# chorowski-lab/pytorch-asr

Hardware: AMD Instinct MI355X
Metric: CTC train-step frames/sec (higher is better)
Workload: dtype bf16; 1 GPU; WSJ mono-char CTC (egs/wsj/yamls/ctc.yaml shapes), DeepSpeech2 conv+4xBiLSTM-320 encoder + FSTDecoder, fwd+bwd+GradientClipping(clip 480000, skip 4.8e+06 = recipe x global_batch/16)+PolyakDecay+Adam, synthetic 40-dim x 1-channel x 1000-frame fbank; batch_per_gpu=768, global_batch=768, frames=1000, classes=49, parallelism=dp1, batch_norm=per-replica statistics, optimizer_steps=142, step_boundary=device: att_speech.fused_step (clip / skip decision + Adam, no read-back)

## Files before the change

### pytorch-asr_amd/csrc/lstm.hip

```cpp
#include "common.h"
#include "../../include/asr_amd.h"
#include "recurrence.h"
#include <stdlib.h>

namespace {

__device__ __forceinline__ void lstm_cell_fwd(const float pre[4], float cprev, float gate[4],
                                              float &c, float &h) {
#pragma clang fp contract(off)
    gate[0] = sigmoidf_(pre[0]);
    gate[1] = sigmoidf_(pre[1]);
    gate[2] = tanhf_(pre[2]);
    gate[3] = sigmoidf_(pre[3]);
    c = gate[1] * cprev + gate[0] * gate[2];
    h = gate[3] * tanhf_(c);
}

typedef float f32x2 __attribute__((ext_vector_type(2)));
__device__ __forceinline__ f32x2 sigmoid2_(f32x2 x) {
#pragma clang fp contract(off)
    const f32x2 t = x * -1.4426950408889634f;
    f32x2 e = {__builtin_amdgcn_exp2f(t.x), __builtin_amdgcn_exp2f(t.y)};
    e = e + 1.f;
    return f32x2{__builtin_amdgcn_rcpf(e.x), __builtin_amdgcn_rcpf(e.y)};
}
__device__ __forceinline__ f32x2 tanh2_(f32x2 x) {
#pragma clang fp contract(off)
    const f32x2 t = x * -2.8853900817779268f;
    f32x2 e = {__builtin_amdgcn_exp2f(t.x), __builtin_amdgcn_exp2f(t.y)};
    e = e + 1.f;
    const f32x2 r = {__builtin_amdgcn_rcpf(e.x), __builtin_amdgcn_rcpf(e.y)};
    return r * 2.f - 1.f;
}
__device__ __forceinline__ void lstm_cell_fwd2(const f32x2 pre[4], f32x2 cprev, f32x2 gate[4],
                                               f32x2 &c, f32x2 &h) {
#pragma clang fp contract(off)
    gate[0] = sigmoid2_(pre[0]);
    gate[1] = sigmoid2_(pre[1]);
    gate[2] = tanh2_(pre[2]);
    gate[3] = sigmoid2_(pre[3]);
    c = gate[1] * cprev + gate[0] * gate[2];
    h = gate[3] * tanh2_(c);
}

__device__ __forceinline__ void lstm_cell_bwd(const float g[4], float cs, float cp, float dh,
                                              float dcin, float d[4], float &dcout) {
#pragma clang fp contract(off)
    const float gi = g[0], gf = g[1], gg = g[2], go = g[3];
    const float tc = tanhf_(cs);
    const float dc = dh * go * (1.f - tc * tc) + dcin;
    d[3] = dh * tc * go * (1.f - go);
    d[0] = dc * gg * gi * (1.f - gi);
    d[1] = dc * cp * gf * (1.f - gf);
    d[2] = dc * gi * (1.f - gg * gg);
    dcout = dc * gf;
}

template <int GXB>
__device__ __forceinline__ float load_gx(const void *gx, size_t i) {
    if constexpr (GXB) return (float)((const __bf16 *)gx)[i];
    else return ((const float *)gx)[i];
}

struct LstmFwdParams {
    const void *gx;
    int gx_bf16;
    const __bf16 *x;
    const __bf16 *wih;
    const __bf16 *whh;
    const int32_t *lens;
    int T, B, H;
    __bf16 *hbuf;
    float *cbuf;
    float *y;
    __bf16 *ybf;
    u32x2 *gates;
    float *csave;
    int step;
    int s_begin, s_end;
    __bf16 *xsum;
};


#ifdef ASR_LSTM_STAMPS
#define STAMP(i) stamp[i] = __builtin_amdgcn_s_memtime()
#else
#define STAMP(i) do {} while (0)
#endif

template <int KS, int BT, int GXB>
__global__ __launch_bounds__(256) void lstm_fwd_step_kernel(LstmFwdParams p) {
#ifdef ASR_LSTM_STAMPS
    unsigned long long stamp[4];
    const unsigned long long stamp_start = __builtin_amdgcn_s_memtime();
#endif
    __shared__ __attribute__((aligned(16))) __bf16 a_lds[BT * KS * 512];
    __shared__ float g_lds[BT][4][32][33];
    const int H = p.H, B = p.B;
    const int j0 = blockIdx.x * 32, b0 = blockIdx.y * 32 * BT, dir = blockIdx.z;
    const int wave = threadIdx.x >> 6, lane = threadIdx.x & 63;
    const int t = dir == 0 ? p.step : p.T - 1 - p.step;
    const int Bp = (B + 63) & ~63;
    const __bf16 *hprev = p.hbuf + ((size_t)(p.step & 1) * 2 + dir) * Bp * H;
    __bf16 *hnext = p.hbuf + ((size_t)((p.step + 1) & 1) * 2 + dir) * Bp * H;

    bf16x8 fb[KS];
    {
        const __bf16 *bp = p.whh + ((size_t)(dir * 4 + wave) * H * H) +
// ... 69 lines not shown
        const int bt = rowg >> 5, row = rowg & 31;
        const int b = b0 + rowg, j = j0 + col;
        if (b < B) {
            const size_t sidx = ((size_t)dir * B + b) * H + j;
            float *yo = p.y + (((size_t)t * B + b) * 2 + dir) * H + j;
            __bf16 *ybo = p.ybf + (((size_t)dir * (p.T + 2) + t + 1) * B + b) * H + j;
            const size_t csv = (((size_t)t * 2 + dir) * B + b) * H + j;
            if (pact[e]) {
                float pre[4], gt[4], c, h;
#pragma unroll
                for (int g = 0; g < 4; ++g) pre[g] = g_lds[bt][g][row][col] + pgx[e][g];
                lstm_cell_fwd(pre, pc[e], gt, c, h);
                p.cbuf[sidx] = c;
                hnext[frag_off(b, j, KS)] = (__bf16)h;
                if (p.y) *yo = h;
                *ybo = (__bf16)h;
                p.gates[csv] = pack_gates(gt);
                p.csave[csv] = c;
            } else {
                hnext[frag_off(b, j, KS)] = hprev[frag_off(b, j, KS)];
                if (p.y) *yo = 0.f;
                *ybo = (__bf16)0.f;
                p.csave[csv] = pc[e];
            }
        }
    }
    STAMP(3);
#ifdef ASR_LSTM_STAMPS
    __syncthreads();
    if (threadIdx.x == 0 && b0 < B) {
        float *o = p.y + (((size_t)t * B + b0) * 2 + dir) * H + j0;
        o[0] = (float)(stamp[0] - stamp_start);
        for (int i = 1; i < 4; ++i) o[i] = (float)(stamp[i] - stamp[i - 1]);
    }
#endif
}

struct LstmBwdParams {
    const float *dy;
    int dy_shared;
    const __bf16 *wihT;
    float *dx;
    const __bf16 *whhT;
    const int32_t *lens;
    int T, B, H;
    const u32x2 *gates;
    const float *csave;
    __bf16 *dgbuf;
    float *dcbuf;
    __bf16 *dgates;
    int step;
};

template <int KS, int BT>
__global__ __launch_bounds__(256) void lstm_bwd_step_kernel(LstmBwdParams p) {
    __shared__ float part[BT][4][32][33];
    const int H = p.H, B = p.B, H4 = 4 * p.H;
    const int j0 = blockIdx.x * 32, b0 = blockIdx.y * 32 * BT, dir = blockIdx.z;
    const int wave = threadIdx.x >> 6, lane = threadIdx.x & 63;
    const int t = dir == 0 ? p.T - 1 - p.step : p.step;
    const int Bp = (B + 63) & ~63;
    constexpr int KS4 = 4 * KS;
    const __bf16 *dgprev = p.dgbuf + ((size_t)(p.step & 1) * 2 + dir) * Bp * H4;
    __bf16 *dgnext = p.dgbuf + ((size_t)((p.step + 1) & 1) * 2 + dir) * Bp * H4;

    bf16x8 fb[KS], fa[BT][KS];
    {
        const __bf16 *bp = p.whhT + (size_t)dir * H * H4 +
                           (((size_t)blockIdx.x * KS4 + (size_t)wave * KS) * 64 + lane) * 8;
#pragma unroll
        for (int k = 0; k < KS; ++k) fb[k] = *reinterpret_cast<const bf16x8 *>(bp + k * 512);
#pragma unroll
        for (int bt = 0; bt < BT; ++bt) {
            const __bf16 *ap = dgprev + ((((size_t)blockIdx.y * BT + bt) * KS4 +
                                          (size_t)wave * KS) * 64 + lane) * 8;
#pragma unroll
            for (int k = 0; k < KS; ++k)
                fa[bt][k] = *reinterpret_cast<const bf16x8 *>(ap + k * 512);
        }
    }

    constexpr int NE = 4 * BT;
    float pg[NE][4], pcs[NE], pcp[NE], pdy[NE], pdc[NE];
    bool pact[NE];
#pragma unroll
    for (int e = 0; e < NE; ++e) {
        const int idx = e * 256 + threadIdx.x;
        const int b = b0 + (idx >> 5), j = j0 + (idx & 31);
        const int bc = b < B ? b : B - 1;
        const int len = p.lens[bc];
        pact[e] = b < B && t < len;
        unpack_gates(p.gates[(((size_t)t * 2 + dir) * B + bc) * H + j], pg[e]);
        pcs[e] = p.csave[(((size_t)t * 2 + dir) * B + bc) * H + j];
        const int tp = dir == 0 ? t - 1 : t + 1;
        const int tpc = tp < 0 ? 0 : (tp >= p.T ? p.T - 1 : tp);
        const float cpv = p.csave[(((size_t)tpc * 2 + dir) * B + bc) * H + j];
        pcp[e] = (tp >= 0 && tp < len) ? cpv : 0.f;
        pdy[e] = p.dy[p.dy_shared ? ((size_t)t * B + bc) * H + j : (((size_t)t * B + bc) * 2 + dir) * H + j];
        pdc[e] = p.dcbuf[((size_t)dir * B + bc) * H + j];
    }

    {
        const int col = lane & 31;
#pragma unroll
        for (int bt = 0; bt < BT; ++bt) {
            f32x16 acc;
#pragma unroll
            for (int i = 0; i < 16; ++i) acc[i] = 0.f;
#pragma unroll
            for (int k = 0; k < KS; ++k)
                acc = __builtin_amdgcn_mfma_f32_32x32x16_bf16(fa[bt][k], fb[k], acc, 0, 0, 0);
#pragma unroll
            for (int i = 0; i < 16; ++i) {
                const int row = (i & 3) + 8 * (i >> 2) + 4 * (lane >> 5);
                part[bt][wave][row][col] = acc[i];
            }
        }
    }
    __syncthreads();

#pragma unroll
    for (int e = 0; e < NE; ++e) {
        const int idx = e * 256 + threadIdx.x;
        const int rowg = idx >> 5, col = idx & 31;
        const int bt = rowg >> 5, row = rowg & 31;
        const int b = b0 + rowg, j = j0 + col;
        if (b < B) {
            const size_t sidx = ((size_t)dir * B + b) * H + j;
            __bf16 *dgo = p.dgates + (((size_t)t * B + b) * 2 + dir) * H4 + j;
            if (pact[e]) {
                const float dh = pdy[e] + (part[bt][0][row][col] + part[bt][1][row][col]) +
                                 (part[bt][2][row][col] + part[bt][3][row][col]);
                float d[4], dcout;
                lstm_cell_bwd(pg[e], pcs[e], pcp[e], dh, pdc[e], d, dcout);
                const float d_i = d[0], d_f = d[1], d_g = d[2], d_o = d[3];
                p.dcbuf[sidx] = dcout;
                dgo[0] = (__bf16)d_i; dgo[H] = (__bf16)d_f;
                dgo[2 * H] = (__bf16)d_g; dgo[3 * H] = (__bf16)d_o;
                dgnext[frag_off(b, j, KS4)] = (__bf16)d_i;
                dgnext[frag_off(b, H + j, KS4)] = (__bf16)d_f;
                dgnext[frag_off(b, 2 * H + j, KS4)] = (__bf16)d_g;
                dgnext[frag_off(b, 3 * H + j, KS4)] = (__bf16)d_o;
            } else {
                p.dcbuf[sidx] = 0.f;
                dgo[0] = (__bf16)0.f; dgo[H] = (__bf16)0.f;
                dgo[2 * H] = (__bf16)0.f; dgo[3 * H] = (__bf16)0.f;
                dgnext[frag_off(b, j, KS4)] = (__bf16)0.f;
                dgnext[frag_off(b, H + j, KS4)] = (__bf16)0.f;
                dgnext[frag_off(b, 2 * H + j, KS4)] = (__bf16)0.f;
                dgnext[frag_off(b, 3 * H + j, KS4)] = (__bf16)0.f;
            }
        }
    }
}


#ifdef ASR_LSTM_STAMPS
#define PSTAMP_DECL unsigned long long pst[6] = {0, 0, 0, 0, 0, 0}, plast = __builtin_amdgcn_s_memtime()
#define PSTAMP(i) do { const unsigned long long now_ = __builtin_amdgcn_s_memtime(); \
                       pst[i] += now_ - plast; plast = now_; } while (0)
#else
#define PSTAMP_DECL do {} while (0)
#define PSTAMP(i) do {} while (0)
#endif

typedef __attribute__((ext_vector_type(4))) int rsrc_words;
__device__ __forceinline__ rsrc_words raw_rsrc(const void *base, unsigned bytes) {
    const unsigned long long a = (unsigned long long)base;
    rsrc_words r;
    r.x = __builtin_amdgcn_readfirstlane((int)(unsigned)a);
    r.y = __builtin_amdgcn_readfirstlane((int)((unsigned)(a >> 32) & 0xffffu));
    r.z = __builtin_amdgcn_readfirstlane((int)bytes);
    r.w = 0x00020000;
    return r;
}
__device__ __forceinline__ void dma16_s(rsrc_words r, unsigned lds_byte, unsigned voff, unsigned soff) {
    unsigned keep;
    asm volatile("s_mov_b32 %0, m0\n\ts_mov_b32 m0, %1\n\ts_nop 0\n\t"
                 "buffer_load_dwordx4 %2, %3, %4 offen lds\n\ts_mov_b32 m0, %0"
                 : "=&s"(keep)
                 : "s"(lds_byte), "v"(voff), "s"(r), "s"(soff)
                 : "memory");
}
__device__ __forceinline__ void dma16_sc1(rsrc_words r, unsigned lds_byte, unsigned voff, unsigned soff) {
    unsigned keep;
// ... 360 lines not shown
                    pre[g] = f32x2{g_lds[g][row][col], g_lds[g][row + 8][col]};
                    if constexpr (!XF) pre[g] = pre[g] + f32x2{pgx[XF ? 0 : e][g], pgx[XF ? 0 : e + 1][g]};
                }
                lstm_cell_fwd2(pre, f32x2{c[e], c[e + 1]}, og, cn, hn);
                const float og0[4] = {og[0].x, og[1].x, og[2].x, og[3].x}, og1[4] = {og[0].y, og[1].y, og[2].y, og[3].y};
                sog[e] = pack_gates(og0);
                sog[e + 1] = pack_gates(og1);
                c[e] = cn.x; c[e + 1] = cn.y;
                soh[e] = dead ? __builtin_nanf("") : hn.x;
                soh[e + 1] = dead ? __builtin_nanf("") : hn.y;
                hq[e] = (__bf16)soh[e]; hq[e + 1] = (__bf16)soh[e + 1];
                shq[e] = hq[e]; shq[e + 1] = hq[e + 1];
            } else {
                cell_one(e);
                if (e + 1 < NE) cell_one(e + 1);
            }
        }
#pragma unroll
        for (int e = 0; e < NE; ++e) {
            const int row = e * 8 + wave;
            sc[e] = c[e];
            h_lds[(((col >> 4) * 64) + row + 32 * ((col >> 3) & 1)) * 8 + (col & 7)] = hq[e];
        }
        __syncthreads();
        if (wave < 4) {
            const u32x4 v = reinterpret_cast<const u32x4 *>(h_lds)[wave * 64 + lane];
            const unsigned off = (unsigned)(((((size_t)((step + 1) & 1) * 2 + dir) * Bp * H) +
                                             ((size_t)btile * KS + 4 * jt + wave) * 512 + lane * 8) * 2);
            __builtin_amdgcn_raw_buffer_store_b128(v, hres, (lane & 31) < 8 * NE ? off : 0xFFFFFFFFu,
                                                   0, ASR_SC1);
        }
        PSTAMP(3);
        bulk_store(true);
        asm volatile("s_waitcnt vmcnt(%0)" ::"n"((NOY ? 3 : 4) * NE) : "memory");
        __syncthreads();
        PSTAMP(4);
        if (tid == 0) __hip_atomic_fetch_add(myctr, 1u, __ATOMIC_RELAXED, __HIP_MEMORY_SCOPE_AGENT);
        if constexpr (summ) sum_store();
        if constexpr (!XF) {
#pragma unroll
            for (int e = 0; e < NE; ++e)
#pragma unroll
                for (int g = 0; g < 4; ++g) pgx[e][g] = ngx[e][g];
        }
        PSTAMP(5);
    }
#ifdef ASR_LSTM_STAMPS
    __syncthreads();
    if (tid == 0 && b0 < B)
        for (int i = 0; i < 6; ++i) p.y[(((size_t)0 * B + b0) * 2 + dir) * H + j0 + i] = (float)pst[i] / T;
#endif
}

template <int KS, int NE>
__global__ __launch_bounds__(512) void lstm_bwd_persist_kernel(LstmBwdParams p, LstmTeamCtl ctl) {
    extern __shared__ __attribute__((aligned(16))) unsigned char smem[];
    constexpr int KS4 = 4 * KS;
    __bf16 *a_lds = reinterpret_cast<__bf16 *>(smem);
    float (*part)[32][65] = reinterpret_cast<float (*)[32][65]>(smem + KS4 * 1024);
    __bf16 *dg_lds = reinterpret_cast<__bf16 *>(smem + KS4 * 1024 + ASR_GLDS_BYTES);
    __shared__ int dead_s;
    const int H = p.H, B = p.B, T = p.T, H4 = 4 * p.H;
    int jt = blockIdx.x, btile = blockIdx.y + ctl.bt0, dir = blockIdx.z;
    if (ctl.xcd_teams) {
        const int slot = blockIdx.x >> 3, team = (slot / (p.H / 64)) * 8 + (blockIdx.x & 7);
        if (team >= ctl.xcd_teams) return;
        jt = slot % (p.H / 64);
        btile = (team >> 1) + ctl.bt0;
        dir = team & 1;
    }
    const int j0 = jt * 64, b0 = btile * (8 * NE), njt = H / 64;
    const int tid = threadIdx.x, wave = tid >> 6, lane = tid & 63;
    const int kq = wave >> 1, js = wave & 1;
    const size_t Bp = ctl.rows;
    unsigned *myctr = ctl.ctr + ((size_t)dir * ctl.nbt + btile) * 32;
    if (tid == 0) dead_s = 0;
    for (int i = tid; i < 8192; i += 512) dg_lds[i] = (__bf16)0.f;
    for (int i = tid; i < KS4 * 64; i += 512)
        reinterpret_cast<u32x4 *>(a_lds)[i] = u32x4{0u, 0u, 0u, 0u};

    bf16x8 fb[KS];
    {
        const __bf16 *bp = p.whhT + (size_t)dir * H * H4 +
                           (((size_t)(2 * jt + js) * KS4 + (size_t)kq * KS) * 64 + lane) * 8;
#pragma unroll
        for (int k = 0; k < KS; ++k) fb[k] = *reinterpret_cast<const bf16x8 *>(bp + k * 512);
    }
    const __amdgpu_buffer_rsrc_t dres = __builtin_amdgcn_make_buffer_rsrc(
        p.dgbuf, 0, (int)(2 * 2 * Bp * H4 * 2), 0x00020000);

    const int col = lane, j = j0 + col;
    float dcarry[NE];
    int len[NE], bcl[NE];
#pragma unroll
    for (int e = 0; e < NE; ++e) {
        const int b = b0 + e * 8 + wave;
        dcarry[e] = 0.f;
        len[e] = b < B ? p.lens[b] : 0;
        bcl[e] = b < B ? b : B - 1;
    }

    typedef unsigned int u32;
    constexpr u32 OOBV = 0xFFFFFFFFu;
    u32 vcs[NE], vdy[NE], vdg[NE];
#pragma unroll
    for (int e = 0; e < NE; ++e) {
        const int b = b0 + e * 8 + wave;
        vcs[e] = (u32)((dir * B + bcl[e]) * H + j) * 4u;
        vdy[e] = (u32)(p.dy_shared ? bcl[e] * H + j : (bcl[e] * 2 + dir) * H + j) * 4u;
        vdg[e] = b < B ? (u32)((b * 2 + dir) * H4 + j) * 2u : OOBV;
    }
    const u32 fg = (u32)B * 2u * H * 8u, fcs = (u32)B * 2u * H * 4u;
    const u32 fdy = (u32)B * H * 4u * (p.dy_shared ? 1u : 2u), fdg = (u32)B * 2u * H4 * 2u;
    const u32 dy2 = p.dy_shared == 2 ? (u32)T * fdy : 0x80000000u;
    const __amdgpu_buffer_rsrc_t gR = __builtin_amdgcn_make_buffer_rsrc(
        const_cast<u32x2 *>(p.gates), 0, (int)((u32)T * fg), 0x00020000);
    const __amdgpu_buffer_rsrc_t csR = __builtin_amdgcn_make_buffer_rsrc(
        const_cast<float *>(p.csave), 0, (int)((u32)T * fcs), 0x00020000);
    const __amdgpu_buffer_rsrc_t dyR = __builtin_amdgcn_make_buffer_rsrc(
        const_cast<float *>(p.dy), 0,
        __builtin_amdgcn_readfirstlane((int)((u32)T * fdy * (p.dy_shared == 2 ? 2u : 1u))), 0x00020000);
    const __amdgpu_buffer_rsrc_t dgR = __builtin_amdgcn_make_buffer_rsrc(
        p.dgates, 0, (int)((u32)T * fdg), 0x00020000);
    auto ldf = [&](__amdgpu_buffer_rsrc_t R, u32 voff, u32 soff) -> float {
        return __builtin_bit_cast(float, __builtin_amdgcn_raw_buffer_load_b32(R, voff, soff, 0));
    };
    struct Pre { u32x2 g[NE]; float cp[NE], dy[NE], dyb[NE]; };
    auto fetch = [&](int t, Pre &q) {
        const int tp = dir == 0 ? t - 1 : t + 1;
        const int tpc = tp < 0 ? 0 : (tp >= T ? T - 1 : tp);
#pragma unroll
        for (int e = 0; e < NE; ++e) {
            q.g[e] = __builtin_amdgcn_raw_buffer_load_b64(gR, vcs[e] * 2u, (u32)t * fg, 0);
            q.cp[e] = ldf(csR, vcs[e], (u32)tpc * fcs);
            q.dy[e] = ldf(dyR, vdy[e], (u32)t * fdy);
            q.dyb[e] = ldf(dyR, vdy[e], (u32)t * fdy + dy2);
        }
    };
    Pre cur;
    float pcs[NE];
    {
        const int t0 = dir == 0 ? T - 1 : 0;
        fetch(t0, cur);
#pragma unroll
        for (int e = 0; e < NE; ++e) pcs[e] = ldf(csR, vcs[e], (u32)t0 * fcs);
    }
    __bf16 sod[NE][4] = {};
    int st = 0;
    auto bulk_store = [&](bool live) {
#pragma unroll
        for (int e = 0; e < NE; ++e)
#pragma unroll
            for (int g = 0; g < 4; ++g)
                __builtin_amdgcn_raw_buffer_store_b16(
                    (short)__builtin_bit_cast(unsigned short, sod[e][g]), dgR, live ? vdg[e] : OOBV,
                    (u32)st * fdg + (u32)g * H * 2u, 0);
    };

    PSTAMP_DECL;
    for (int step = 0; step < T; ++step) {
        const int t = dir == 0 ? T - 1 - step : step;
        if (step > 0 && tid == 0 && !dead_s) {
            if (!team_wait(myctr, (unsigned)(njt * step), ctl.spin_limit, ctl.err)) dead_s = 1;
        }
        PSTAMP(0);
        __syncthreads();
        constexpr int RL = 8 * NE, CPK = 2 * RL;
        constexpr int CHO = (KS4 - 16) * CPK, NI = (CHO + 511) / 512;
        u32x4 tmp[NI > 0 ? NI : 1];
        if constexpr (NI > 0) {
            const unsigned base = (unsigned)((((size_t)(step & 1) * 2 + dir) * Bp * H4 +
                                              (size_t)btile * KS4 * 512) * 2);
#pragma unroll
            for (int i = 0; i < NI; ++i) {
                const int co = i * 512 + tid;
                const int cc = co < CHO ? co : CHO - 1;
                const int kq = cc / CPK, q = cc - kq * CPK, g = kq / (KS - 4), r = kq - g * (KS - 4);
                const int k = g * KS + (r < 4 * jt ? r : r + 4);
                tmp[i] = __builtin_amdgcn_raw_buffer_load_b128(
                    dres, base + (k * 64 + (q < RL ? q : q + (32 - RL))) * 16, 0, ASR_SC1);
            }
        }
        bulk_store(step > 0);
#pragma unroll
        for (int i = 0; i < 2; ++i) {
            const int c = i * 512 + tid, bi = c >> 6;
            reinterpret_cast<u32x4 *>(a_lds)[((bi >> 2) * KS + 4 * jt + (bi & 3)) * 64 + (c & 63)] =
                reinterpret_cast<const u32x4 *>(dg_lds)[c];
        }
        if constexpr (NI > 0) {
#pragma unroll
            for (int i = 0; i < NI; ++i) {
                const int co = i * 512 + tid;
                const int kq = co / CPK, q = co - kq * CPK, g = kq / (KS - 4), r = kq - g * (KS - 4);
                const int k = g * KS + (r < 4 * jt ? r : r + 4);
                if (co < CHO)
                    reinterpret_cast<u32x4 *>(a_lds)[k * 64 + (q < RL ? q : q + (32 - RL))] = tmp[i];
            }
        }
        __syncthreads();
        PSTAMP(1);
        Pre nxt;
        {
            const int sn = step + 1 < T ? step + 1 : step;
            fetch(dir == 0 ? T - 1 - sn : sn, nxt);
        }
        {
            f32x16 acc;
#pragma unroll
            for (int i = 0; i < 16; ++i) acc[i] = 0.f;
            const bf16x8 *al = reinterpret_cast<const bf16x8 *>(a_lds) + (size_t)kq * KS * 64 + lane;
            acc = mfma_chain<0, KS, 4>(al, fb, acc);
            const int c32 = lane & 31;
#pragma unroll
            for (int i = 0; i < 16; ++i) {
                const int row = (i & 3) + 8 * (i >> 2) + 4 * (lane >> 5);
                part[kq][row][js * 32 + c32] = acc[i];
            }
        }
        __syncthreads();
        PSTAMP(2);
        const bool dead = dead_s != 0;
        st = t;
        const int tp = dir == 0 ? t - 1 : t + 1;
#pragma unroll
        for (int e = 0; e < NE; ++e) {
            const int row = e * 8 + wave;
            float od[4];
            if (t < len[e]) {
                const float dh = (cur.dy[e] + cur.dyb[e]) + (part[0][row][col] + part[1][row][col]) +
                                 (part[2][row][col] + part[3][row][col]);
                const float cp = (tp >= 0 && tp < len[e]) ? cur.cp[e] : 0.f;
                float dcout, gt[4];
                unpack_gates(cur.g[e], gt);
                lstm_cell_bwd(gt, pcs[e], cp, dh, dcarry[e], od, dcout);
                dcarry[e] = dcout;
                if (dead) od[0] = od[1] = od[2] = od[3] = __builtin_nanf("");
            } else {
                od[0] = od[1] = od[2] = od[3] = 0.f;
                dcarry[e] = 0.f;
            }
            const int slot = ((col >> 4) * 64 + row + 32 * ((col >> 3) & 1)) * 8 + (col & 7);
#pragma unroll
            for (int g = 0; g < 4; ++g) {
                sod[e][g] = (__bf16)od[g];
                dg_lds[g * 2048 + slot] = sod[e][g];
            }
            pcs[e] = cur.cp[e];
        }
        __syncthreads();
#pragma unroll
        for (int r = 0; r < 2; ++r) {
            const int bi = wave * 2 + r, g = bi >> 2, kk = bi & 3;
            const u32x4 v = reinterpret_cast<const u32x4 *>(dg_lds)[bi * 64 + lane];
            const unsigned off = (unsigned)(((((size_t)((step + 1) & 1) * 2 + dir) * Bp * H4) +
                                             ((size_t)btile * KS4 + g * KS + 4 * jt + kk) * 512 + lane * 8) * 2);
            __builtin_amdgcn_raw_buffer_store_b128(v, dres, (lane & 31) < 8 * NE ? off : 0xFFFFFFFFu,
                                                   0, ASR_SC1);
        }
        PSTAMP(3);
        asm volatile("s_waitcnt vmcnt(0)" ::: "memory");
        __syncthreads();
        PSTAMP(4);
        if (tid == 0) __hip_atomic_fetch_add(myctr, 1u, __ATOMIC_RELAXED, __HIP_MEMORY_SCOPE_AGENT);
        cur = nxt;
        PSTAMP(5);
    }
    if (T > 0) bulk_store(true);
#ifdef ASR_LSTM_STAMPS
    __syncthreads();
    if (tid == 0 && b0 < B)
        for (int i = 0; i < 6; ++i)
            p.dgates[(((size_t)0 * B + b0) * 2 + dir) * H4 + j0 + i] = (__bf16)((float)pst[i] / T / 16.f);
#endif
}

template <int KS, int NE>
__global__ __launch_bounds__(512) void lstm_bwd_dx_kernel(LstmBwdParams p, LstmTeamCtl ctl) {
    extern __shared__ __attribute__((aligned(16))) unsigned char smem[];
    constexpr int KS4 = 4 * KS, RL = 8 * NE;
    __bf16 *a_lds = reinterpret_cast<__bf16 *>(smem);
    float (*part)[32][65] = reinterpret_cast<float (*)[32][65]>(smem + KS4 * 1024);
    __bf16 *dg_lds = reinterpret_cast<__bf16 *>(smem + KS4 * 1024 + ASR_GLDS_BYTES);
    unsigned char *pre = smem + KS4 * 1024 + ASR_GLDS_BYTES + 16384;
    u32x2 (*pg)[64] = reinterpret_cast<u32x2 (*)[64]>(pre);
    float (*pcp)[64] = reinterpret_cast<float (*)[64]>(pre + RL * 512);
    float (*pdy)[64] = reinterpret_cast<float (*)[64]>(pre + RL * 768);
    __shared__ int dead_s;
    typedef unsigned int u32;
    constexpr u32 OOBV = 0x80000000u;
    const int H = p.H, B = p.B, T = p.T, H4 = 4 * p.H;
    int jt = blockIdx.x, btile = blockIdx.y + ctl.bt0, dir = blockIdx.z;
    if (ctl.xcd_teams) {
        const int slot = blockIdx.x >> 3, team = (slot / (p.H / 64)) * 8 + (blockIdx.x & 7);
        if (team >= ctl.xcd_teams) return;
        jt = slot % (p.H / 64);
        btile = (team >> 1) + ctl.bt0;
        dir = team & 1;
    }
    const int j0 = jt * 64, b0 = btile * RL, njt = H / 64;
    const int tid = threadIdx.x, lane = tid & 63;
    const int wave = __builtin_amdgcn_readfirstlane(tid >> 6);
    const int kq = wave >> 1, js = wave & 1;
    const size_t Bp = ctl.rows;
    unsigned *myctr = ctl.ctr + ((size_t)dir * ctl.nbt + btile) * 32;
    if (tid == 0) dead_s = 0;
    for (int i = tid; i < 8192; i += 512) dg_lds[i] = (__bf16)0.f;
    for (int i = tid; i < KS4 * 64; i += 512)
        reinterpret_cast<u32x4 *>(a_lds)[i] = u32x4{0u, 0u, 0u, 0u};

    bf16x8 fb[KS], fxb[KS];
    {
        const size_t wo = (size_t)dir * H * H4 +
                          (((size_t)(2 * jt + js) * KS4 + (size_t)kq * KS) * 64 + lane) * 8;
#pragma unroll
        for (int k = 0; k < KS; ++k) fb[k] = *reinterpret_cast<const bf16x8 *>(p.whhT + wo + k * 512);
#pragma unroll
        for (int k = 0; k < KS; ++k) fxb[k] = *reinterpret_cast<const bf16x8 *>(p.wihT + wo + k * 512);
    }
    const __amdgpu_buffer_rsrc_t dres = __builtin_amdgcn_make_buffer_rsrc(
        p.dgbuf, 0, (int)(2 * 2 * Bp * H4 * 2), 0x00020000);
    const rsrc_words dresD = raw_rsrc(p.dgbuf, (unsigned)(2 * 2 * Bp * H4 * 2));

    const int col = lane;
    int len[NE], bc[NE];
    bool inb[NE];
    float dcarry[NE], pcs[NE];
#pragma unroll
    for (int e = 0; e < NE; ++e) {
        const int b = b0 + e * 8 + wave;
        inb[e] = b < B;
        bc[e] = b < B ? b : B - 1;
        len[e] = __builtin_amdgcn_readfirstlane(b < B ? p.lens[bc[e]] : 0);
        dcarry[e] = 0.f;
    }
    const u32 l4 = (u32)lane * 4u, l2 = (u32)lane * 2u;
    const u32 fg = (u32)B * 2u * H * 8u, fcs = (u32)B * 2u * H * 4u;
    const u32 fdy = (u32)B * H * 4u * (p.dy_shared ? 1u : 2u), fdg = (u32)B * 2u * H4 * 2u;
    const u32 fdx = (u32)B * H * 4u;
    const rsrc_words gD = raw_rsrc(p.gates, (u32)T * fg);
    const rsrc_words csD = raw_rsrc(p.csave, (u32)T * fcs);
    const rsrc_words dyD = raw_rsrc(p.dy, (u32)T * fdy * (p.dy_shared == 2 ? 2u : 1u));
    const __amdgpu_buffer_rsrc_t dgR = __builtin_amdgcn_make_buffer_rsrc(
        p.dgates, 0, (int)((u32)T * fdg), 0x00020000);
    const __amdgpu_buffer_rsrc_t dxR = __builtin_amdgcn_make_buffer_rsrc(
        p.dx, 0, (int)(2u * (u32)T * fdx), 0x00020000);

    constexpr int NQ = 5 * RL / 4, NQW = (NQ + 7) / 8;
    u32 pvo[NQW];
#pragma unroll
    for (int i = 0; i < NQW; ++i) {
        const int q = wave + 8 * i;
        if (q < RL / 2) {
            const int r = 2 * q + (lane >> 5), b = b0 + r < B ? b0 + r : B - 1;
            pvo[i] = (u32)((dir * B + b) * H + j0) * 8u + (u32)(lane & 31) * 16u;
        } else {
            const int qq = q < 3 * RL / 4 ? q - RL / 2 : (q < RL ? q - 3 * RL / 4 : q - RL);
            const int r = 4 * qq + (lane >> 4), b = b0 + r < B ? b0 + r : B - 1;
            if (q < 3 * RL / 4) pvo[i] = (u32)((dir * B + b) * H + j0) * 4u + (u32)(lane & 15) * 16u;
            else pvo[i] = (u32)(p.dy_shared ? b * H + j0 : (b * 2 + dir) * H + j0) * 4u + (u32)(lane & 15) * 16u;
            if (q >= RL && p.dy_shared != 2) pvo[i] = OOBV;
        }
    }
    auto pre_dma = [&](int t) {
        const int tp = dir == 0 ? t - 1 : t + 1;
        const int tpc = tp < 0 ? 0 : (tp >= T ? T - 1 : tp);
#pragma unroll
        for (int i = 0; i < NQW; ++i) {
            const int q = wave + 8 * i;
// ... 67 lines not shown
    {
        const int t0 = dir == 0 ? T - 1 : 0;
#pragma unroll
        for (int e = 0; e < NE; ++e)
            pcs[e] = p.csave[(((size_t)t0 * 2 + dir) * B + bc[e]) * H + j0 + col];
    }
    const bool last_q = wave + 8 * (NQW - 1) < NQ;
#pragma unroll
    for (int k = 0; k < KS; ++k) {
        asm volatile("" : "+v"(fb[k]));
        asm volatile("" : "+v"(fxb[k]));
    }
#pragma unroll
    for (int e = 0; e < NE; ++e) asm volatile("" : "+v"(pcs[e]));

    PSTAMP_DECL;
    for (int step = 0; step < T; ++step) {
        const int t = dir == 0 ? T - 1 - step : step;
        const unsigned target = (unsigned)(njt * step);
        const bool poller = step > 0 && tid == 0 && !dead_s;
        unsigned seen = 0;
        if (poller) seen = __hip_atomic_load(myctr, __ATOMIC_RELAXED, __HIP_MEMORY_SCOPE_AGENT);
        if (step >= 2) {
            f32x16 acc;
#pragma unroll
            for (int i = 0; i < 16; ++i) acc[i] = 0.f;
            const bf16x8 *al = reinterpret_cast<const bf16x8 *>(a_lds) + (size_t)kq * KS * 64 + lane;
            acc = mfma_chain<0, KS / 2, 2>(al, fxb, acc);
            if (poller && seen < target)
                seen = __hip_atomic_load(myctr, __ATOMIC_RELAXED, __HIP_MEMORY_SCOPE_AGENT);
            acc = mfma_chain<KS / 2, KS, 2>(al, fxb, acc);
            const int c32 = lane & 31;
#pragma unroll
            for (int i = 0; i < 16; ++i) {
                const int row = (i & 3) + 8 * (i >> 2) + 4 * (lane >> 5);
                part[kq][row][js * 32 + c32] = acc[i];
            }
        }
        if (poller && seen < target) {
            if (!team_wait(myctr, target, ctl.spin_limit, ctl.err)) dead_s = 1;
        }
        PSTAMP(0);
        __syncthreads();
        tile_dma(step);
        bulk_store(step > 0);
        own_copy();
        dx_store(step >= 2, step - 2);
        pre_dma(t);
        if (last_q) asm volatile("s_waitcnt vmcnt(%0)" ::"n"(5 * NE + NQW) : "memory");
        else asm volatile("s_waitcnt vmcnt(%0)" ::"n"(5 * NE + NQW - 1) : "memory");
        __syncthreads();
        PSTAMP(1);
        {
            f32x16 acc;
#pragma unroll
            for (int i = 0; i < 16; ++i) acc[i] = 0.f;
            const bf16x8 *al = reinterpret_cast<const bf16x8 *>(a_lds) + (size_t)kq * KS * 64 + lane;
            acc = mfma_chain<0, KS, 2>(al, fb, acc);
            const int c32 = lane & 31;
#pragma unroll
            for (int i = 0; i < 16; ++i) {
                const int row = (i & 3) + 8 * (i >> 2) + 4 * (lane >> 5);
                part[kq][row][js * 32 + c32] = acc[i];
            }
        }
        asm volatile("s_waitcnt vmcnt(0)" ::: "memory");
        __syncthreads();
        PSTAMP(2);
        const bool dead = dead_s != 0;
        st = t;
        const int tp = dir == 0 ? t - 1 : t + 1;
#pragma unroll
        for (int e = 0; e < NE; ++e) {
            const int row = e * 8 + wave;
            float od[4];
            const float cpn = pcp[row][col];
            if (t < len[e]) {
                const float dh = (pdy[row][col] + pdy[RL + row][col]) +
                                 (part[0][row][col] + part[1][row][col]) +
                                 (part[2][row][col] + part[3][row][col]);
                const float cp = (tp >= 0 && tp < len[e]) ? cpn : 0.f;
                float dcout, gt[4];
                unpack_gates(pg[row][col], gt);
                lstm_cell_bwd(gt, pcs[e], cp, dh, dcarry[e], od, dcout);
                dcarry[e] = dcout;
                if (dead) od[0] = od[1] = od[2] = od[3] = __builtin_nanf("");
            } else {
                od[0] = od[1] = od[2] = od[3] = 0.f;
                dcarry[e] = 0.f;
            }
            const int slot = ((col >> 4) * 64 + row + 32 * ((col >> 3) & 1)) * 8 + (col & 7);
#pragma unroll
            for (int g = 0; g < 4; ++g) {
                sod[e][g] = (__bf16)od[g];
                dg_lds[g * 2048 + slot] = sod[e][g];
            }
            pcs[e] = cpn;
        }
        __syncthreads();
#pragma unroll
        for (int r = 0; r < 2; ++r) {
            const int bi = wave * 2 + r, g = bi >> 2, kk = bi & 3;
            const u32x4 v = reinterpret_cast<const u32x4 *>(dg_lds)[bi * 64 + lane];
            const unsigned off = (unsigned)(((((size_t)((step + 1) & 1) * 2 + dir) * Bp * H4) +
                                             ((size_t)btile * KS4 + g * KS + 4 * jt + kk) * 512 + lane * 8) * 2);
            __builtin_amdgcn_raw_buffer_store_b128(v, dres, (lane & 31) < RL ? off : 0xFFFFFFFFu,
                                                   0, ASR_SC1);
        }
        PSTAMP(3);
        asm volatile("s_waitcnt vmcnt(0)" ::: "memory");
        __syncthreads();
        PSTAMP(4);
        if (tid == 0) __hip_atomic_fetch_add(myctr, 1u, __ATOMIC_RELAXED, __HIP_MEMORY_SCOPE_AGENT);
        PSTAMP(5);
    }
    bulk_store(true);
    if (T >= 2) dx_mfma();
    if (tid == 0 && !dead_s) {
        if (!team_wait(myctr, (unsigned)(njt * T), ctl.spin_limit, ctl.err)) dead_s = 1;
    }
    __syncthreads();
    tile_dma(T);
    own_copy();
    dx_store(T >= 2, T - 2);
    asm volatile("s_waitcnt vmcnt(%0)" ::"n"(NE) : "memory");
    __syncthreads();
    dx_mfma();
    __syncthreads();
    dx_store(true, T - 1);
#ifdef ASR_LSTM_STAMPS
    __syncthreads();
    if (tid == 0 && b0 < B)
        for (int i = 0; i < 6; ++i)
// ... 189 lines not shown
    return lstm_bwd_impl(dy, dy_shared, whhT_bf16, wihT_bf16, lens, T, B, H, gates_bf16, csave,
                         dgates_bf16, dx, workspace, workspace_bytes, err_flag, stream);
}
#endif

namespace {
int lstm_bwd_impl(const float *dy, int dy_shared, const void *whhT_bf16, const void *wihT_bf16,
                  const int32_t *lens, int T, int B, int H, const void *gates_bf16,
                  const float *csave, void *dgates_bf16, float *dx, void *workspace,
                  int64_t workspace_bytes, uint32_t *err_flag, void *stream) {
    const bool fused = wihT_bf16 != nullptr;
    if (T < 0 || B <= 0 || H <= 0 || (H % 32) != 0 || dy_shared < 0 || dy_shared > 2) return ASR_EINVAL;
    if (T == 0) return ASR_OK;
    if (!dy || !whhT_bf16 || !lens || !gates_bf16 || !csave || !dgates_bf16 || !workspace)
        return ASR_EINVAL;
    if (fused && !(asr_lstm_fused_supported(B, H, H) & 2)) return ASR_EUNSUPPORTED;
    if (workspace_bytes < asr_lstm_workspace_bytes(B, H)) return ASR_EINVAL;
    hipStream_t s = (hipStream_t)stream;
    LstmBwdParams p;
    const size_t Bp = (size_t)plane_rows(B);
    const size_t dbytes = (size_t)2 * 2 * Bp * 4 * H * 2, cbytes = (size_t)2 * B * H * 4;
    __bf16 *wpack = (__bf16 *)((char *)workspace + dbytes + cbytes);
    p.dy = dy; p.dy_shared = dy_shared; p.whhT = wpack; p.lens = lens;
    p.wihT = wpack + (size_t)2 * H * 4 * H; p.dx = dx;
    p.T = T; p.B = B; p.H = H;
    p.gates = (const u32x2 *)gates_bf16; p.csave = csave;
    p.dgbuf = (__bf16 *)workspace;
    p.dcbuf = (float *)((char *)workspace + dbytes);
    p.dgates = (__bf16 *)dgates_bf16;
    {
        ZeroList zl;
        zl.add(workspace, dbytes + cbytes);
        if (persist_enabled())
            zl.add((char *)workspace + asr_lstm_workspace_bytes(B, H) - ctl_bytes(B), (size_t)ctl_bytes(B));
        zl.launch(s);
    }
    hipLaunchKernelGGL(lstm_pack_kernel, dim3(1024), dim3(256), 0, s,
                       (const __bf16 *)whhT_bf16, wpack, 2, H, 4 * H, 0);
    if (fused)
        hipLaunchKernelGGL(lstm_pack_kernel, dim3(1024), dim3(256), 0, s,
                           (const __bf16 *)wihT_bf16, wpack + (size_t)2 * H * 4 * H, 2, H, 4 * H, 0);
    if (persist_enabled()) {
        unsigned *ctl_words = (unsigned *)((char *)workspace + asr_lstm_workspace_bytes(B, H) - ctl_bytes(B));
        void (*pk[3])(LstmBwdParams, LstmTeamCtl) = {nullptr, nullptr, nullptr};
#define ASR_PICK(KSV) if (H == 16 * KSV && !fused) { pk[0] = lstm_bwd_persist_kernel<KSV, 2>; \
        pk[1] = lstm_bwd_persist_kernel<KSV, 3>; pk[2] = lstm_bwd_persist_kernel<KSV, 4>; }
        ASR_PICK(20) ASR_PICK(4) ASR_PICK(8) ASR_PICK(16) ASR_PICK(24)
#undef ASR_PICK
#define ASR_PICK(KSV) if (H == 16 * KSV && fused) { pk[0] = lstm_bwd_dx_kernel<KSV, 2>; \
        pk[1] = lstm_bwd_dx_kernel<KSV, 3>; }
        ASR_PICK(20) ASR_PICK(4) ASR_PICK(8) ASR_PICK(16)
#undef ASR_PICK
        const bool fits32 = (uint64_t)T * B * 8 * H * 4 < (fused ? (1ull << 31) : (1ull << 32));
        const size_t lds = (size_t)(H / 4) * 1024 + ASR_GLDS_BYTES + 16384 + (fused ? 24 * 1280 : 0);
        if (fits32 && (pk[2] || fused) && launch_persist(pk, p, B, H, lds, ctl_words, err_flag, s))
            return hipGetLastError() == hipSuccess ? ASR_OK : ASR_ELAUNCH;
    }
    if (fused || dy_shared == 2) return ASR_EUNSUPPORTED;
    const int bt = 1;
    const dim3 grid(H / 32, (B + 32 * bt - 1) / (32 * bt), 2);
    void (*kern)(LstmBwdParams) = nullptr;
#define ASR_PICK(KSV)                                                              \
    if (H == 16 * KSV) kern = bt == 2 ? lstm_bwd_step_kernel<KSV, 2> : lstm_bwd_step_kernel<KSV, 1>;
    ASR_PICK(20) ASR_PICK(4) ASR_PICK(8) ASR_PICK(16) ASR_PICK(24) ASR_PICK(32) ASR_PICK(48)
#undef ASR_PICK
    if (!kern) return ASR_EUNSUPPORTED;
    for (int step = 0; step < T; ++step) {
        p.step = step;
        hipLaunchKernelGGL(kern, grid, dim3(256), 0, s, p);
    }
    return hipGetLastError() == hipSuccess ? ASR_OK : ASR_ELAUNCH;
}
}
```

Before: 36.46 million frames/s.

## Split LSTM backward dh recurrence into two k-halves with direct buffer loads

The persistent LSTM backward kernel no longer stages the previous step's dgate fragments through a staging LDS buffer. Each wave now loads the remote part of its k-slice straight from global memory into registers and reads only its locally produced block from LDS. The k-reduction is split into two independent MFMA accumulator chains over eight waves, so dependent MFMAs can overlap. Gate-dependent backward terms are precomputed before the cross-block wait, and the bulk store and next-step fetch are scheduled under the loads. In exchange, more registers and global loads sit on the critical path, the float summation order changes, and the step and dx kernels are reordered to match.

Result: slower. 35.71 million frames/s (-2.1%).

```diff
diff --git a/pytorch-asr_amd/csrc/lstm.hip b/pytorch-asr_amd/csrc/lstm.hip
--- a/pytorch-asr_amd/csrc/lstm.hip
+++ b/pytorch-asr_amd/csrc/lstm.hip
@@ -43,17 +43,35 @@
     h = gate[3] * tanh2_(c);
 }
 
+struct LstmCellBwdPre {
+    float gi, gf, gg, go, cp, tc, omt, omi, omf, omg, omo;
+};
+__device__ __forceinline__ LstmCellBwdPre lstm_cell_bwd_prepare(const float g[4], float cs, float cp) {
+#pragma clang fp contract(off)
+    LstmCellBwdPre q;
+    q.gi = g[0]; q.gf = g[1]; q.gg = g[2]; q.go = g[3];
+    q.cp = cp;
+    q.tc = tanhf_(cs);
+    q.omt = 1.f - q.tc * q.tc;
+    q.omi = 1.f - q.gi;
+    q.omf = 1.f - q.gf;
+    q.omg = 1.f - q.gg * q.gg;
+    q.omo = 1.f - q.go;
+    return q;
+}
+__device__ __forceinline__ void lstm_cell_bwd_finish(const LstmCellBwdPre &q, float dh, float dcin,
+                                                     float d[4], float &dcout) {
+#pragma clang fp contract(off)
+    const float dc = dh * q.go * q.omt + dcin;
+    d[3] = dh * q.tc * q.go * q.omo;
+    d[0] = dc * q.gg * q.gi * q.omi;
+    d[1] = dc * q.cp * q.gf * q.omf;
+    d[2] = dc * q.gi * q.omg;
+    dcout = dc * q.gf;
+}
 __device__ __forceinline__ void lstm_cell_bwd(const float g[4], float cs, float cp, float dh,
                                               float dcin, float d[4], float &dcout) {
-#pragma clang fp contract(off)
-    const float gi = g[0], gf = g[1], gg = g[2], go = g[3];
-    const float tc = tanhf_(cs);
-    const float dc = dh * go * (1.f - tc * tc) + dcin;
-    d[3] = dh * tc * go * (1.f - go);
-    d[0] = dc * gg * gi * (1.f - gi);
-    d[1] = dc * cp * gf * (1.f - gf);
-    d[2] = dc * gi * (1.f - gg * gg);
-    dcout = dc * gf;
+    lstm_cell_bwd_finish(lstm_cell_bwd_prepare(g, cs, cp), dh, dcin, d, dcout);
 }
 
 template <int GXB>
@@ -229,6 +247,28 @@
     int step;
 };
 
+template <int KS>
+struct DhOrder {
+    static_assert(KS % 2 == 0 && KS >= 4, "a gate's k-steps are cut in two halves");
+    static constexpr int HK = KS / 2;
+    int lo, ls, nloc;
+    __device__ __forceinline__ DhOrder(int jt, int kh) {
+        lo = kh * HK;
+        const int a = 4 * jt > lo ? 4 * jt : lo, b = 4 * jt + 4 < lo + HK ? 4 * jt + 4 : lo + HK;
+        nloc = b > a ? b - a : 0;
+        ls = nloc ? a : lo + HK;
+    }
+    __device__ __forceinline__ int kstep(int p) const {
+        if (p < nloc) return ls + p;
+        const int k = lo + p - nloc;
+        return k >= ls ? k + nloc : k;
+    }
+};
+__device__ __forceinline__ float dh_pair(float c0, float c1) { return c0 + c1; }
+__device__ __forceinline__ float dh_sum(float dy, float q0, float q1, float q2, float q3) {
+    return dy + (q0 + q1) + (q2 + q3);
+}
+
 template <int KS, int BT>
 __global__ __launch_bounds__(256) void lstm_bwd_step_kernel(LstmBwdParams p) {
     __shared__ float part[BT][4][32][33];
@@ -237,23 +277,29 @@
     const int wave = threadIdx.x >> 6, lane = threadIdx.x & 63;
     const int t = dir == 0 ? p.T - 1 - p.step : p.step;
     const int Bp = (B + 63) & ~63;
-    constexpr int KS4 = 4 * KS;
+    constexpr int KS4 = 4 * KS, HK = KS / 2;
     const __bf16 *dgprev = p.dgbuf + ((size_t)(p.step & 1) * 2 + dir) * Bp * H4;
     __bf16 *dgnext = p.dgbuf + ((size_t)((p.step + 1) & 1) * 2 + dir) * Bp * H4;
 
     bf16x8 fb[KS], fa[BT][KS];
     {
+        const DhOrder<KS> o0((int)blockIdx.x >> 1, 0), o1((int)blockIdx.x >> 1, 1);
         const __bf16 *bp = p.whhT + (size_t)dir * H * H4 +
                            (((size_t)blockIdx.x * KS4 + (size_t)wave * KS) * 64 + lane) * 8;
 #pragma unroll
-        for (int k = 0; k < KS; ++k) fb[k] = *reinterpret_cast<const bf16x8 *>(bp + k * 512);
+        for (int c = 0; c < KS; ++c) {
+            const int k = c < HK ? o0.kstep(c) : o1.kstep(c - HK);
+            fb[c] = *reinterpret_cast<const bf16x8 *>(bp + k * 512);
+        }
 #pragma unroll
         for (int bt = 0; bt < BT; ++bt) {
             const __bf16 *ap = dgprev + ((((size_t)blockIdx.y * BT + bt) * KS4 +
                                           (size_t)wave * KS) * 64 + lane) * 8;
 #pragma unroll
-            for (int k = 0; k < KS; ++k)
-                fa[bt][k] = *reinterpret_cast<const bf16x8 *>(ap + k * 512);
+            for (int c = 0; c < KS; ++c) {
+                const int k = c < HK ? o0.kstep(c) : o1.kstep(c - HK);
+                fa[bt][c] = *reinterpret_cast<const bf16x8 *>(ap + k * 512);
+            }
         }
     }
 
@@ -281,16 +327,18 @@
         const int col = lane & 31;
 #pragma unroll
         for (int bt = 0; bt < BT; ++bt) {
-            f32x16 acc;
-#pragma unroll
-            for (int i = 0; i < 16; ++i) acc[i] = 0.f;
-#pragma unroll
-            for (int k = 0; k < KS; ++k)
-                acc = __builtin_amdgcn_mfma_f32_32x32x16_bf16(fa[bt][k], fb[k], acc, 0, 0, 0);
+            f32x16 acc0, acc1;
+#pragma unroll
+            for (int i = 0; i < 16; ++i) acc0[i] = acc1[i] = 0.f;
+#pragma unroll
+            for (int c = 0; c < HK; ++c) {
+                acc0 = __builtin_amdgcn_mfma_f32_32x32x16_bf16(fa[bt][c], fb[c], acc0, 0, 0, 0);
+                acc1 = __builtin_amdgcn_mfma_f32_32x32x16_bf16(fa[bt][HK + c], fb[HK + c], acc1, 0, 0, 0);
+            }
 #pragma unroll
             for (int i = 0; i < 16; ++i) {
                 const int row = (i & 3) + 8 * (i >> 2) + 4 * (lane >> 5);
-                part[bt][wave][row][col] = acc[i];
+                part[bt][wave][row][col] = dh_pair(acc0[i], acc1[i]);
             }
         }
     }
@@ -306,8 +354,8 @@
             const size_t sidx = ((size_t)dir * B + b) * H + j;
             __bf16 *dgo = p.dgates + (((size_t)t * B + b) * 2 + dir) * H4 + j;
             if (pact[e]) {
-                const float dh = pdy[e] + (part[bt][0][row][col] + part[bt][1][row][col]) +
-                                 (part[bt][2][row][col] + part[bt][3][row][col]);
+                const float dh = dh_sum(pdy[e], part[bt][0][row][col], part[bt][1][row][col],
+                                        part[bt][2][row][col], part[bt][3][row][col]);
                 float d[4], dcout;
                 lstm_cell_bwd(pg[e], pcs[e], pcp[e], dh, pdc[e], d, dcout);
                 const float d_i = d[0], d_f = d[1], d_g = d[2], d_o = d[3];
@@ -774,13 +822,43 @@
 #endif
 }
 
+template <int HK, int NLOC, typename KOff, typename Under>
+__device__ __forceinline__ void dh_chains(__amdgpu_buffer_rsrc_t dres, unsigned voff, KOff &&koff,
+                                          const bf16x8 *loc, const bf16x8 (&fb)[HK][2],
+                                          f32x16 &acc0, f32x16 &acc1, Under &&under) {
+    constexpr int NR = HK - NLOC;
+    bf16x8 ar[NR > 0 ? NR : 1], al[NLOC > 0 ? NLOC : 1];
+#pragma unroll
+    for (int i = 0; i < NR; ++i)
+        ar[i] = __builtin_bit_cast(bf16x8, __builtin_amdgcn_raw_buffer_load_b128(
+                                               dres, voff, koff(NLOC + i), ASR_SC1));
+    __builtin_amdgcn_sched_barrier(0);
+    under();
+    __builtin_amdgcn_sched_barrier(0);
+#pragma unroll
+    for (int i = 0; i < NLOC; ++i) al[i] = loc[i * 64];
+#pragma unroll
+    for (int i = 0; i < NLOC; ++i) {
+        acc0 = __builtin_amdgcn_mfma_f32_32x32x16_bf16(al[i], fb[i][0], acc0, 0, 0, 0);
+        acc1 = __builtin_amdgcn_mfma_f32_32x32x16_bf16(al[i], fb[i][1], acc1, 0, 0, 0);
+    }
+#pragma unroll
+    for (int i = 0; i < NR; ++i) {
+        acc0 = __builtin_amdgcn_mfma_f32_32x32x16_bf16(ar[i], fb[NLOC + i][0], acc0, 0, 0, 0);
+        acc1 = __builtin_amdgcn_mfma_f32_32x32x16_bf16(ar[i], fb[NLOC + i][1], acc1, 0, 0, 0);
+    }
+    if constexpr (NLOC > 0) __builtin_amdgcn_sched_group_barrier(0x100, NLOC, 0);
+    __builtin_amdgcn_sched_group_barrier(0x008, 2 * HK, 0);
+    __builtin_amdgcn_sched_barrier(0);
+}
+
 template <int KS, int NE>
 __global__ __launch_bounds__(512) void lstm_bwd_persist_kernel(LstmBwdParams p, LstmTeamCtl ctl) {
     extern __shared__ __attribute__((aligned(16))) unsigned char smem[];
-    constexpr int KS4 = 4 * KS;
-    __bf16 *a_lds = reinterpret_cast<__bf16 *>(smem);
-    float (*part)[32][65] = reinterpret_cast<float (*)[32][65]>(smem + KS4 * 1024);
-    __bf16 *dg_lds = reinterpret_cast<__bf16 *>(smem + KS4 * 1024 + ASR_GLDS_BYTES);
+    constexpr int KS4 = 4 * KS, HK = KS / 2, RL = 8 * NE;
+    constexpr bool EARLY = KS <= 20;
+    float (*part)[32][65] = reinterpret_cast<float (*)[32][65]>(smem);
+    __bf16 *dg_lds = reinterpret_cast<__bf16 *>(smem + 2 * ASR_GLDS_BYTES);
     __shared__ int dead_s;
     const int H = p.H, B = p.B, T = p.T, H4 = 4 * p.H;
     int jt = blockIdx.x, btile = blockIdx.y + ctl.bt0, dir = blockIdx.z;
@@ -791,23 +869,24 @@
         btile = (team >> 1) + ctl.bt0;
         dir = team & 1;
     }
-    const int j0 = jt * 64, b0 = btile * (8 * NE), njt = H / 64;
-    const int tid = threadIdx.x, wave = tid >> 6, lane = tid & 63;
-    const int kq = wave >> 1, js = wave & 1;
+    const int j0 = jt * 64, b0 = btile * RL, njt = H / 64;
+    const int tid = threadIdx.x, lane = tid & 63;
+    const int wave = __builtin_amdgcn_readfirstlane(tid >> 6);
+    const int kg = wave >> 1, kh = wave & 1;
+    const DhOrder<KS> ord(jt, kh);
     const size_t Bp = ctl.rows;
     unsigned *myctr = ctl.ctr + ((size_t)dir * ctl.nbt + btile) * 32;
     if (tid == 0) dead_s = 0;
     for (int i = tid; i < 8192; i += 512) dg_lds[i] = (__bf16)0.f;
-    for (int i = tid; i < KS4 * 64; i += 512)
-        reinterpret_cast<u32x4 *>(a_lds)[i] = u32x4{0u, 0u, 0u, 0u};
-
-    bf16x8 fb[KS];
-    {
-        const __bf16 *bp = p.whhT + (size_t)dir * H * H4 +
-                           (((size_t)(2 * jt + js) * KS4 + (size_t)kq * KS) * 64 + lane) * 8;
-#pragma unroll
-        for (int k = 0; k < KS; ++k) fb[k] = *reinterpret_cast<const bf16x8 *>(bp + k * 512);
-    }
+
+    bf16x8 fb[HK][2];
+#pragma unroll
+    for (int c = 0; c < HK; ++c)
+#pragma unroll
+        for (int n = 0; n < 2; ++n)
+            fb[c][n] = *reinterpret_cast<const bf16x8 *>(
+                p.whhT + (size_t)dir * H * H4 +
+                (((size_t)(2 * jt + n) * KS4 + (size_t)kg * KS + ord.kstep(c)) * 64 + lane) * 8);
     const __amdgpu_buffer_rsrc_t dres = __builtin_amdgcn_make_buffer_rsrc(
         p.dgbuf, 0, (int)(2 * 2 * Bp * H4 * 2), 0x00020000);
 
@@ -878,84 +957,78 @@
                     (short)__builtin_bit_cast(unsigned short, sod[e][g]), dgR, live ? vdg[e] : OOBV,
                     (u32)st * fdg + (u32)g * H * 2u, 0);
     };
+    const u32 avo = (lane & 31) < RL ? (u32)lane * 16u : OOBV;
+    const bf16x8 *loc = reinterpret_cast<const bf16x8 *>(dg_lds) +
+                        (size_t)(kg * 4 + (ord.ls - 4 * jt)) * 64 + lane;
 
     PSTAMP_DECL;
     for (int step = 0; step < T; ++step) {
         const int t = dir == 0 ? T - 1 - step : step;
+        const int tp = dir == 0 ? t - 1 : t + 1;
+        LstmCellBwdPre cq[NE];
+        float dys[NE];
+        Pre nxt;
+        auto prepare = [&]() {
+#pragma unroll
+            for (int e = 0; e < NE; ++e) {
+                float gt[4];
+                unpack_gates(cur.g[e], gt);
+                cq[e] = lstm_cell_bwd_prepare(gt, pcs[e], (tp >= 0 && tp < len[e]) ? cur.cp[e] : 0.f);
+                dys[e] = cur.dy[e] + cur.dyb[e];
+                pcs[e] = cur.cp[e];
+                if constexpr (EARLY) {
+                    asm volatile("" : "+v"(cq[e].tc), "+v"(cq[e].omt), "+v"(dys[e]));
+                }
+            }
+        };
+        if constexpr (EARLY) prepare();
         if (step > 0 && tid == 0 && !dead_s) {
             if (!team_wait(myctr, (unsigned)(njt * step), ctl.spin_limit, ctl.err)) dead_s = 1;
         }
         PSTAMP(0);
         __syncthreads();
-        constexpr int RL = 8 * NE, CPK = 2 * RL;
-        constexpr int CHO = (KS4 - 16) * CPK, NI = (CHO + 511) / 512;
-        u32x4 tmp[NI > 0 ? NI : 1];
-        if constexpr (NI > 0) {
+        PSTAMP(1);
+        {
             const unsigned base = (unsigned)((((size_t)(step & 1) * 2 + dir) * Bp * H4 +
                                               (size_t)btile * KS4 * 512) * 2);
-#pragma unroll
-            for (int i = 0; i < NI; ++i) {
-                const int co = i * 512 + tid;
-                const int cc = co < CHO ? co : CHO - 1;
-                const int kq = cc / CPK, q = cc - kq * CPK, g = kq / (KS - 4), r = kq - g * (KS - 4);
-                const int k = g * KS + (r < 4 * jt ? r : r + 4);
-                tmp[i] = __builtin_amdgcn_raw_buffer_load_b128(
-                    dres, base + (k * 64 + (q < RL ? q : q + (32 - RL))) * 16, 0, ASR_SC1);
-            }
-        }
-        bulk_store(step > 0);
-#pragma unroll
-        for (int i = 0; i < 2; ++i) {
-            const int c = i * 512 + tid, bi = c >> 6;
-            reinterpret_cast<u32x4 *>(a_lds)[((bi >> 2) * KS + 4 * jt + (bi & 3)) * 64 + (c & 63)] =
-                reinterpret_cast<const u32x4 *>(dg_lds)[c];
-        }
-        if constexpr (NI > 0) {
-#pragma unroll
-            for (int i = 0; i < NI; ++i) {
-                const int co = i * 512 + tid;
-                const int kq = co / CPK, q = co - kq * CPK, g = kq / (KS - 4), r = kq - g * (KS - 4);
-                const int k = g * KS + (r < 4 * jt ? r : r + 4);
-                if (co < CHO)
-                    reinterpret_cast<u32x4 *>(a_lds)[k * 64 + (q < RL ? q : q + (32 - RL))] = tmp[i];
-            }
-        }
-        __syncthreads();
-        PSTAMP(1);
-        Pre nxt;
-        {
-            const int sn = step + 1 < T ? step + 1 : step;
-            fetch(dir == 0 ? T - 1 - sn : sn, nxt);
-        }
-        {
-            f32x16 acc;
-#pragma unroll
-            for (int i = 0; i < 16; ++i) acc[i] = 0.f;
-            const bf16x8 *al = reinterpret_cast<const bf16x8 *>(a_lds) + (size_t)kq * KS * 64 + lane;
-            acc = mfma_chain<0, KS, 4>(al, fb, acc);
+            auto koff = [&](int c) -> unsigned { return base + (unsigned)(kg * KS + ord.kstep(c)) * 1024u; };
+            const int sn = step + 1 < T ? step + 1 : step, tn = dir == 0 ? T - 1 - sn : sn;
+            auto under = [&]() {
+                bulk_store(step > 0);
+                if constexpr (EARLY) fetch(tn, cur);
+            };
+            f32x16 acc0, acc1;
+#pragma unroll
+            for (int i = 0; i < 16; ++i) acc0[i] = acc1[i] = 0.f;
+            if (HK % 4 != 0 && ord.nloc == 2) dh_chains<HK, 2>(dres, avo, koff, loc, fb, acc0, acc1, under);
+            else if (HK >= 4 && ord.nloc == 4) dh_chains<HK, (HK >= 4 ? 4 : 0)>(dres, avo, koff, loc, fb, acc0, acc1, under);
+            else dh_chains<HK, 0>(dres, avo, koff, loc, fb, acc0, acc1, under);
             const int c32 = lane & 31;
 #pragma unroll
             for (int i = 0; i < 16; ++i) {
                 const int row = (i & 3) + 8 * (i >> 2) + 4 * (lane >> 5);
-                part[kq][row][js * 32 + c32] = acc[i];
-            }
+                part[wave][row][c32] = acc0[i];
+                part[wave][row][32 + c32] = acc1[i];
+            }
+            if constexpr (!EARLY) fetch(tn, nxt);
         }
         __syncthreads();
         PSTAMP(2);
         const bool dead = dead_s != 0;
         st = t;
-        const int tp = dir == 0 ? t - 1 : t + 1;
+        if constexpr (!EARLY) { prepare(); cur = nxt; }
 #pragma unroll
         for (int e = 0; e < NE; ++e) {
             const int row = e * 8 + wave;
             float od[4];
             if (t < len[e]) {
-                const float dh = (cur.dy[e] + cur.dyb[e]) + (part[0][row][col] + part[1][row][col]) +
-                                 (part[2][row][col] + part[3][row][col]);
-                const float cp = (tp >= 0 && tp < len[e]) ? cur.cp[e] : 0.f;
-                float dcout, gt[4];
-                unpack_gates(cur.g[e], gt);
-                lstm_cell_bwd(gt, pcs[e], cp, dh, dcarry[e], od, dcout);
+                const float dh = dh_sum(dys[e],
+                                        dh_pair(part[0][row][col], part[1][row][col]),
+                                        dh_pair(part[2][row][col], part[3][row][col]),
+                                        dh_pair(part[4][row][col], part[5][row][col]),
+                                        dh_pair(part[6][row][col], part[7][row][col]));
+                float dcout;
+                lstm_cell_bwd_finish(cq[e], dh, dcarry[e], od, dcout);
                 dcarry[e] = dcout;
                 if (dead) od[0] = od[1] = od[2] = od[3] = __builtin_nanf("");
             } else {
@@ -968,7 +1041,6 @@
                 sod[e][g] = (__bf16)od[g];
                 dg_lds[g * 2048 + slot] = sod[e][g];
             }
-            pcs[e] = cur.cp[e];
         }
         __syncthreads();
 #pragma unroll
@@ -977,7 +1049,7 @@
             const u32x4 v = reinterpret_cast<const u32x4 *>(dg_lds)[bi * 64 + lane];
             const unsigned off = (unsigned)(((((size_t)((step + 1) & 1) * 2 + dir) * Bp * H4) +
                                              ((size_t)btile * KS4 + g * KS + 4 * jt + kk) * 512 + lane * 8) * 2);
-            __builtin_amdgcn_raw_buffer_store_b128(v, dres, (lane & 31) < 8 * NE ? off : 0xFFFFFFFFu,
+            __builtin_amdgcn_raw_buffer_store_b128(v, dres, (lane & 31) < RL ? off : 0xFFFFFFFFu,
                                                    0, ASR_SC1);
         }
         PSTAMP(3);
@@ -985,7 +1057,6 @@
         __syncthreads();
         PSTAMP(4);
         if (tid == 0) __hip_atomic_fetch_add(myctr, 1u, __ATOMIC_RELAXED, __HIP_MEMORY_SCOPE_AGENT);
-        cur = nxt;
         PSTAMP(5);
     }
     if (T > 0) bulk_store(true);
@@ -1000,7 +1071,7 @@
 template <int KS, int NE>
 __global__ __launch_bounds__(512) void lstm_bwd_dx_kernel(LstmBwdParams p, LstmTeamCtl ctl) {
     extern __shared__ __attribute__((aligned(16))) unsigned char smem[];
-    constexpr int KS4 = 4 * KS, RL = 8 * NE;
+    constexpr int KS4 = 4 * KS, RL = 8 * NE, HK = KS / 2;
     __bf16 *a_lds = reinterpret_cast<__bf16 *>(smem);
     float (*part)[32][65] = reinterpret_cast<float (*)[32][65]>(smem + KS4 * 1024);
     __bf16 *dg_lds = reinterpret_cast<__bf16 *>(smem + KS4 * 1024 + ASR_GLDS_BYTES);
@@ -1024,6 +1095,7 @@
     const int tid = threadIdx.x, lane = tid & 63;
     const int wave = __builtin_amdgcn_readfirstlane(tid >> 6);
     const int kq = wave >> 1, js = wave & 1;
+    const DhOrder<KS> ord0(jt, 0), ord1(jt, 1);
     const size_t Bp = ctl.rows;
     unsigned *myctr = ctl.ctr + ((size_t)dir * ctl.nbt + btile) * 32;
     if (tid == 0) dead_s = 0;
@@ -1036,7 +1108,9 @@
         const size_t wo = (size_t)dir * H * H4 +
                           (((size_t)(2 * jt + js) * KS4 + (size_t)kq * KS) * 64 + lane) * 8;
 #pragma unroll
-        for (int k = 0; k < KS; ++k) fb[k] = *reinterpret_cast<const bf16x8 *>(p.whhT + wo + k * 512);
+        for (int c = 0; c < KS; ++c)
+            fb[c] = *reinterpret_cast<const bf16x8 *>(
+                p.whhT + wo + (c < HK ? ord0.kstep(c) : ord1.kstep(c - HK)) * 512);
 #pragma unroll
         for (int k = 0; k < KS; ++k) fxb[k] = *reinterpret_cast<const bf16x8 *>(p.wihT + wo + k * 512);
     }
@@ -1210,16 +1284,20 @@
         __syncthreads();
         PSTAMP(1);
         {
-            f32x16 acc;
-#pragma unroll
-            for (int i = 0; i < 16; ++i) acc[i] = 0.f;
+            f32x16 acc0, acc1;
+#pragma unroll
+            for (int i = 0; i < 16; ++i) acc0[i] = acc1[i] = 0.f;
             const bf16x8 *al = reinterpret_cast<const bf16x8 *>(a_lds) + (size_t)kq * KS * 64 + lane;
-            acc = mfma_chain<0, KS, 2>(al, fb, acc);
+#pragma unroll
+            for (int c = 0; c < HK; ++c) {
+                acc0 = __builtin_amdgcn_mfma_f32_32x32x16_bf16(al[ord0.kstep(c) * 64], fb[c], acc0, 0, 0, 0);
+                acc1 = __builtin_amdgcn_mfma_f32_32x32x16_bf16(al[ord1.kstep(c) * 64], fb[HK + c], acc1, 0, 0, 0);
+            }
             const int c32 = lane & 31;
 #pragma unroll
             for (int i = 0; i < 16; ++i) {
                 const int row = (i & 3) + 8 * (i >> 2) + 4 * (lane >> 5);
-                part[kq][row][js * 32 + c32] = acc[i];
+                part[kq][row][js * 32 + c32] = dh_pair(acc0[i], acc1[i]);
             }
         }
         asm volatile("s_waitcnt vmcnt(0)" ::: "memory");
@@ -1234,9 +1312,8 @@
             float od[4];
             const float cpn = pcp[row][col];
             if (t < len[e]) {
-                const float dh = (pdy[row][col] + pdy[RL + row][col]) +
-                                 (part[0][row][col] + part[1][row][col]) +
-                                 (part[2][row][col] + part[3][row][col]);
+                const float dh = dh_sum(pdy[row][col] + pdy[RL + row][col], part[0][row][col],
+                                        part[1][row][col], part[2][row][col], part[3][row][col]);
                 const float cp = (tp >= 0 && tp < len[e]) ? cpn : 0.f;
                 float dcout, gt[4];
                 unpack_gates(pg[row][col], gt);
@@ -1532,7 +1609,8 @@
         ASR_PICK(20) ASR_PICK(4) ASR_PICK(8) ASR_PICK(16)
 #undef ASR_PICK
         const bool fits32 = (uint64_t)T * B * 8 * H * 4 < (fused ? (1ull << 31) : (1ull << 32));
-        const size_t lds = (size_t)(H / 4) * 1024 + ASR_GLDS_BYTES + 16384 + (fused ? 24 * 1280 : 0);
+        const size_t lds = fused ? (size_t)(H / 4) * 1024 + ASR_GLDS_BYTES + 16384 + 24 * 1280
+                                 : (size_t)2 * ASR_GLDS_BYTES + 16384;
         if (fits32 && (pk[2] || fused) && launch_persist(pk, p, B, H, lds, ctl_words, err_flag, s))
             return hipGetLastError() == hipSuccess ? ASR_OK : ASR_ELAUNCH;
     }
```
